# alibaba/animate-anything

Measured on AMD Instinct MI355X. Metric: UNet3D denoising steps/sec @16fx512x512 bs=1, higher is better.
Workload: dtype fp16; 1 GPU; animate_anything_512_v1.02 UNet3D (1413M params, seeded random init), 16 frames x 512x512, pipeline bs=1 per GPU (CFG batch 2, 17 frames inside), DPM-Solver++ step, hipGraph=on; clips_per_gpu=1, clips=1, parallelism=clip-sharded x1, collective=none

## Files before the change

animate_anything_amd/csrc/aa_api.hip:

```cpp
#include "aa_launch.h"

namespace aa { thread_local hipError_t g_lds_error = hipSuccess; }

static const char* aa_post_launch() {
    hipError_t e = hipGetLastError();
    if (e == hipSuccess && aa::g_lds_error != hipSuccess) { e = aa::g_lds_error; aa::g_lds_error = hipSuccess; }
    return e == hipSuccess ? nullptr : hipGetErrorString(e);
}
#define AA_POST_LAUNCH() aa_post_launch()

#include "aa_api_impl.h"
```

animate_anything_amd/csrc/aa_api_impl.h:

```cpp
#pragma once
#include <stdarg.h>
#include <stdio.h>
#include <stdlib.h>
#include "aa_mi355.h"
#include "kernels/conv_gemm.h"
#include "kernels/conv_gemm_dma.h"
#include "kernels/conv_slab.h"
#include "kernels/conv_gemm_x.h"
#include "kernels/norm.h"
#include "kernels/attention.h"
#include "kernels/seq_attention.h"
#include "kernels/ff_fused.h"
#include "kernels/linear_rows.h"
#include "kernels/linear_fp8.h"
#include "kernels/glue.h"

namespace aa {

static thread_local char g_err[512] = "";

static int fail(int code, const char* fmt, ...) {
    va_list ap;
    va_start(ap, fmt);
    vsnprintf(g_err, sizeof(g_err), fmt, ap);
    va_end(ap);
    return code;
}

static int finish(const char* what) {
    const char* e = AA_POST_LAUNCH();
    if (e) return fail(AA_E_HIP, "%s: %s", what, e);
    return AA_OK;
}

static bool aligned16(const void* p) { return (reinterpret_cast<uintptr_t>(p) & 15) == 0; }

struct CgCfg { int bm, bn, wm, wn, bk, stages, per_cu; float rate; int slab = 0; int x = 0; int sched = 0; };
constexpr int cg_dp(int dp3, int dp0, int dp1) { return (dp3 | dp0 << 4 | dp1 << 8) << 6; }
static const CgCfg kCgCfgs[] = {
    {128, 64, 2, 2, 64, 2, 3, 0.78f},
    {128, 128, 2, 2, 64, 2, 2, 0.90f},
    {192, 256, 3, 2, 64, 2, 1, 1.05f},
    {256, 256, 4, 2, 64, 2, 1, 1.10f},
    {256, 320, 4, 2, 64, 2, 1, 1.10f},
    {192, 320, 3, 2, 64, 2, 1, 1.05f},
    {256, 320, 4, 2, 32, 4, 1, 1.15f},
    {256, 256, 4, 2, 32, 4, 1, 1.15f},
    {128, 128, 2, 2, 32, 4, 2, 0.95f},
    {128, 64, 2, 2, 32, 4, 3, 0.80f},
    {192, 320, 3, 2, 32, 4, 1, 1.10f},
    {128, 320, 2, 2, 32, 2, 2, 1.10f},
    {128, 256, 2, 2, 32, 2, 2, 1.05f},
    {128, 256, 2, 2, 64, 2, 1, 1.00f},
    {256, 320, 4, 2, 64, 2, 1, 1.30f, 0, 0, 1},
    {256, 256, 4, 2, 64, 2, 1, 1.25f, 0, 0, 1},
    {128, 128, 2, 2, 32, 2, 3, 0.90f},
    {128, 64, 2, 2, 32, 2, 4, 0.78f},
    {64, 128, 2, 2, 32, 2, 4, 0.70f},
    {64, 64, 2, 2, 32, 2, 6, 0.60f},
    {64, 256, 2, 2, 32, 2, 3, 0.80f},
    {256, 320, 4, 2, 32, 4, 1, 1.20f, 0, 0, 1},
    {256, 256, 4, 2, 32, 4, 1, 1.20f, 0, 0, 1},
    {192, 256, 2, 4, 64, 2, 1, 1.05f},
    {192, 256, 2, 4, 64, 2, 1, 1.05f, 0, 0, 1},
    {128, 256, 2, 4, 32, 2, 2, 1.00f},
    {256, 320, 4, 2, 64, 2, 1, 1.30f, 0, 0, 2},
    {256, 256, 4, 2, 64, 2, 1, 1.25f, 0, 0, 2},
    {192, 256, 2, 4, 64, 2, 1, 1.05f, 0, 0, 2},
    {256, 320, 4, 2, 32, 4, 1, 1.20f, 0, 0, 2},
    {128, 320, 2, 2, 32, 2, 2, 1.10f, 0, 0, 2},
    {128, 128, 2, 2, 64, 2, 2, 0.90f, 0, 0, 2},
    {192, 320, 3, 2, 64, 2, 1, 1.05f, 0, 0, 2},
    {128, 256, 2, 2, 32, 2, 2, 1.05f, 0, 0, 2},
    {256, 320, 4, 2, 32, 3, 1, 1.00f, 1},
    {256, 256, 4, 2, 32, 3, 1, 1.00f, 1},
    {256, 256, 2, 2, 64, 2, 1, 1.45f, 0, 1, cg_dp(8, 8, 0)},
    {256, 320, 2, 2, 64, 2, 1, 1.45f, 0, 1, cg_dp(11, 7, 0)},
    {256, 256, 2, 2, 64, 2, 1, 1.40f, 0, 1, cg_dp(6, 5, 5)},
    {256, 320, 2, 2, 64, 2, 1, 1.40f, 0, 1, cg_dp(7, 6, 5)},
    {256, 256, 4, 2, 64, 2, 1, 1.35f, 0, 1, cg_dp(2, 2, 2)},
    {256, 256, 2, 2, 32, 4, 1, 1.50f, 0, 1, cg_dp(4, 0, 0)},
    {256, 320, 2, 2, 32, 4, 1, 1.50f, 0, 1, cg_dp(5, 0, 0)},
    {256, 256, 4, 2, 32, 4, 1, 1.45f, 0, 1, cg_dp(2, 0, 0)},
    {128, 256, 2, 2, 32, 3, 2, 1.20f, 0, 1, cg_dp(3, 0, 0)},
    {256, 128, 4, 1, 32, 3, 2, 1.20f, 0, 1, cg_dp(3, 0, 0)},
    {192, 256, 2, 2, 64, 2, 1, 1.30f, 0, 1, cg_dp(5, 5, 4)},
    {128, 128, 2, 2, 64, 2, 2, 1.00f, 0, 1, cg_dp(2, 2, 2)},
    {128, 128, 2, 2, 32, 4, 2, 1.00f, 0, 1, cg_dp(2, 0, 0)},
    {192, 320, 2, 2, 64, 2, 1, 1.35f, 0, 1, cg_dp(6, 5, 5)},
};
constexpr int kNumCgCfgs = sizeof(kCgCfgs) / sizeof(kCgCfgs[0]);

static thread_local int g_tile_override = -2;
static int cg_force_cfg() {
    if (g_tile_override == -2) { const char* e = getenv("AA_FORCE_CFG"); g_tile_override = e ? atoi(e) : -1; }
    return g_tile_override;
}

static bool cg_slab_ok(const AaConvGemm& d, const CgCfg& c) {
    const int hw = d.h_in * d.w_in;
    return d.kh == 3 && d.kw == 3 && d.stride == 1 && d.pad_h == 1 && d.pad_w == 1 && d.h_virt == d.h_in && d.w_virt == d.w_in &&
           d.h_out == d.h_in && d.w_out == d.w_in && d.k_order == 1 && d.c0 % 64 == 0 && d.c1 % 64 == 0 && !d.geglu && !d.bias_per_row &&
           c.bm % d.w_in == 0 && hw % c.bm == 0 && (c.bm / d.w_in + 2) * (d.w_in + 2) <= CS_SLAB_ROWS && !(d.debug & 8);
}

static thread_local unsigned g_x_disabled = 0;
static bool cg_x_ok(const AaConvGemm& d) {
    if (!(d.h_virt == d.h_in && d.w_virt == d.w_in)) return false;
    {
        const int taps = d.kh * d.kw;
        if (taps > 1 && d.k_order != 1) return false;
        if (taps > 31) return false;
        const int64_t px = (int64_t)d.n_img * d.h_in * d.w_in + (int64_t)d.pad_h * d.w_in + d.pad_w + (int64_t)d.kh * d.w_in + d.kw;
        if (px >= ((int64_t)1 << 24) || px * (d.c0 > d.c1 ? d.c0 : d.c1) * 2 >= ((int64_t)1 << 31)) return false;
    }
    if (d.rowvec) {
        const int64_t M = (int64_t)d.n_img * d.h_out * d.w_out;
        const int64_t ld = d.rowvec_ld ? d.rowvec_ld : d.n_out;
// ... 558 lines not shown
        AA_LAUNCH((groupnorm_coef_kernel<f16_t>), dim3(d->n_groups_img), dim3(GN_THREADS), lds, stream, *d, (const float*)ws, chunks, coef);
    } else {
        AA_LAUNCH((groupnorm_stats_kernel<bf16_t>), dim3(chunks, d->n_groups_img), dim3(GN_THREADS), (size_t)C * 8 * (1 + rpp), stream, *d, ws, chunks);
        AA_LAUNCH((groupnorm_coef_kernel<bf16_t>), dim3(d->n_groups_img), dim3(GN_THREADS), lds, stream, *d, (const float*)ws, chunks, coef);
    }
    return finish("groupnorm_coef");
}

int aa_layernorm(const void* x, const void* gamma, const void* beta, void* y, int64_t rows, int32_t channels,
                 float eps, int32_t dtype, void* stream) {
    using namespace aa;
    if (rows <= 0 || channels <= 0 || channels % 8 || channels > 2048) return fail(AA_E_SHAPE, "layernorm: rows=%lld channels=%d", (long long)rows, channels);
    if (!aligned16(x) || !aligned16(y) || !aligned16(gamma) || !aligned16(beta)) return fail(AA_E_ALIGN, "layernorm: operands must be 16-byte aligned");
    const int sj = channels <= 512 ? 1 : (channels <= 1024 ? 2 : 4);
    const int per_wg = 4 * (4 / sj);
    const dim3 grid((unsigned)((rows + per_wg - 1) / per_wg)), block(256);
    if (dtype != AA_F16 && dtype != AA_BF16) return fail(AA_E_DTYPE, "layernorm: unsupported dtype %d", dtype);
#define AA_LN(T, SJ) AA_LAUNCH((layernorm_kernel<T, SJ>), grid, block, 0, stream, (const T*)x, (const T*)gamma, (const T*)beta, (T*)y, rows, channels, eps)
    if (dtype == AA_F16) { if (sj == 1) AA_LN(f16_t, 1); else if (sj == 2) AA_LN(f16_t, 2); else AA_LN(f16_t, 4); }
    else                 { if (sj == 1) AA_LN(bf16_t, 1); else if (sj == 2) AA_LN(bf16_t, 2); else AA_LN(bf16_t, 4); }
#undef AA_LN
    return finish("layernorm");
}

int aa_ln_finalize(const float* stats, int32_t parts, float* coef, int64_t rows, int32_t channels, float eps, void* stream) {
    using namespace aa;
    if (!stats || !coef || parts <= 0 || rows <= 0 || channels <= 0) return fail(AA_E_SHAPE, "ln_finalize: rows=%lld parts=%d channels=%d", (long long)rows, parts, channels);
    if (!aligned16(coef)) return fail(AA_E_ALIGN, "ln_finalize: coef must be 16-byte aligned");
    const dim3 grid((unsigned)((rows + 255) / 256)), block(256);
    AA_LAUNCH(ln_finalize_kernel<0>, grid, block, 0, stream, stats, coef, rows, (int)parts, 1.0f / (float)channels, eps);
    return finish("ln_finalize");
}

int aa_attention(const AaAttention* d, void* stream) {
    using namespace aa;
    if (!d) return fail(AA_E_SHAPE, "attention: null descriptor");
    if (d->head_dim != 64 && d->head_dim != 8 && d->head_dim != 80) return fail(AA_E_SHAPE, "attention: head_dim must be 64, 8 or 80 (got %d)", d->head_dim);
    if (d->q_len <= 0 || d->kv_len <= 0 || d->heads <= 0 || d->n_outer <= 0 || d->n_inner <= 0) return fail(AA_E_SHAPE, "attention: bad lengths");
    const AaAttnOperand* ops[4] = {&d->q, &d->k, &d->v, &d->o};
    for (const AaAttnOperand* x : ops) {
        if (!aligned16(x->ptr) || x->ld % 8 || x->col0 % 8) return fail(AA_E_ALIGN, "attention: operand rows must be 16-byte aligned");
        if (x->outer_div <= 0) return fail(AA_E_SHAPE, "attention: outer_div must be >= 1");
        if (x->seq_mod < 0) return fail(AA_E_SHAPE, "attention: seq_mod must be >= 0");
    }
    if (d->q.seq_mod || d->o.seq_mod) return fail(AA_E_SHAPE, "attention: seq_mod addressing is for K / V only");
    if (d->causal && d->head_dim != 64) return fail(AA_E_SHAPE, "attention: causal masking is implemented for head_dim 64");
    if (d->head_dim == 64 && (attn_extent_bytes(d->k, d->n_outer, d->n_inner, d->kv_len) >= ((int64_t)1 << 31) ||
        attn_extent_bytes(d->v, d->n_outer, d->n_inner, d->kv_len) >= ((int64_t)1 << 31)))
        return fail(AA_E_SHAPE, "attention: K / V operand must stay below 2 GiB");
    if (d->dtype == AA_F16) return attention_t<f16_t>(*d, stream);
    if (d->dtype == AA_BF16) return attention_t<bf16_t>(*d, stream);
    return fail(AA_E_DTYPE, "attention: unsupported dtype %d", d->dtype);
}

int aa_seq_self_attention_ok(const AaSeqSelfAttn* d) {
    using namespace aa;
    if (!d) return 0;
    if (d->channels != 320 && d->channels != 512 && d->channels != 640) return 0;
    if (d->seq_len < 1 || d->seq_len > 32 || d->n_outer <= 0 || d->n_inner <= 0) return 0;
    if (d->ldx % 8 || d->ldo % 8 || d->ldx < d->channels || d->ldo < d->channels) return 0;
    if (d->x_bytes <= 0 || d->o_bytes <= 0 || d->x_bytes >= ((int64_t)1 << 31) || d->o_bytes >= ((int64_t)1 << 31)) return 0;
    if (d->dtype != AA_F16 && d->dtype != AA_BF16) return 0;
    return 1;
}

int aa_seq_self_attention(const AaSeqSelfAttn* d, void* stream) {
    using namespace aa;
    if (!d) return fail(AA_E_SHAPE, "seq_self_attention: null descriptor");
    if (!aa_seq_self_attention_ok(d))
        return fail(AA_E_SHAPE, "seq_self_attention: unsupported call (channels %d, seq_len %d, ldx %d, ldo %d, dtype %d)", d->channels, d->seq_len, d->ldx, d->ldo, d->dtype);
    if (!aligned16(d->x) || !aligned16(d->w) || !aligned16(d->o) || !aligned16(d->w_bias))
        return fail(AA_E_ALIGN, "seq_self_attention: operands must be 16-byte aligned");
    if (d->normalize && !(d->ln_eps > 0.0f)) return fail(AA_E_SHAPE, "seq_self_attention: normalize needs ln_eps > 0");
    if (d->pre_w) {
        if (!d->pre_out || !aligned16(d->pre_w) || !aligned16(d->pre_out) || !aligned16(d->pre_bias) || !aligned16(d->pre_residual))
            return fail(AA_E_ALIGN, "seq_self_attention: the projection in front needs pre_out and 16-byte aligned operands");
        const int64_t rows_ext = d->x_bytes / (2 * (int64_t)d->ldx);
        if (d->ld_pre % 8 || d->ld_pre < d->channels || rows_ext * d->ld_pre * 2 >= ((int64_t)1 << 31) ||
            (d->pre_residual && (d->ld_res % 8 || d->ld_res < d->channels || rows_ext * d->ld_res * 2 >= ((int64_t)1 << 31))))
            return fail(AA_E_SHAPE, "seq_self_attention: bad row pitch / extent of pre_out / pre_residual");
    } else if (d->pre_bias || d->pre_residual || d->pre_out) return fail(AA_E_SHAPE, "seq_self_attention: pre_bias / pre_residual / pre_out without pre_w");
    const int per = (32 * SA_NW) / d->seq_len;
    const int64_t n_seq = (int64_t)d->n_outer * d->n_inner;
    const dim3 grid((unsigned)((n_seq + per - 1) / per)), block(64 * SA_NW);
    const size_t lds = sa_lds_bytes(d->channels);
#define AA_SA(T, C_) AA_LAUNCH((seq_self_attention_kernel<T, C_>), grid, block, lds, stream, *d)
    if (d->dtype == AA_F16) {
        if (d->channels == 320) AA_SA(f16_t, 320); else if (d->channels == 512) AA_SA(f16_t, 512); else AA_SA(f16_t, 640);
    } else {
        if (d->channels == 320) AA_SA(bf16_t, 320); else if (d->channels == 512) AA_SA(bf16_t, 512); else AA_SA(bf16_t, 640);
    }
#undef AA_SA
    return finish("seq_self_attention");
}

int aa_ff_fused_ok(const AaFFFused* d) {
    if (!d || d->channels != 320 || d->rows <= 0) return 0;
    if (d->ldx % 8 || d->ldo % 8 || d->ld_outer % 8 || d->ldx < d->channels || d->ldo < d->channels || (d->outer && d->ld_outer < d->channels)) return 0;
    const int64_t lim = (int64_t)1 << 31;
    if (d->rows * d->ldx * 2 >= lim || d->rows * d->ldo * 2 >= lim || (d->outer && d->rows * d->ld_outer * 2 >= lim)) return 0;
    if (d->dtype != AA_F16 && d->dtype != AA_BF16) return 0;
    return 1;
}

int aa_ff_fused(const AaFFFused* d, void* stream) {
    using namespace aa;
    if (!d) return fail(AA_E_SHAPE, "ff_fused: null descriptor");
    if (!aa_ff_fused_ok(d)) return fail(AA_E_SHAPE, "ff_fused: unsupported call (channels %d, rows %lld, dtype %d)", d->channels, (long long)d->rows, d->dtype);
    if (!d->x || !d->out || !d->w) return fail(AA_E_SHAPE, "ff_fused: x, out, w are required");
    if (!aligned16(d->x) || !aligned16(d->outer) || !aligned16(d->out) || !aligned16(d->w)) return fail(AA_E_ALIGN, "ff_fused: operands must be 16-byte aligned");
    if (d->normalize && !(d->ln_eps > 0.0f)) return fail(AA_E_SHAPE, "ff_fused: normalize needs ln_eps > 0");
    const dim3 grid((unsigned)((d->rows + 32 * FF_NW - 1) / (32 * FF_NW))), block(64 * FF_NW);
    const int abl = d->flags >> 8;
#define AA_FF(ABL_) case ABL_: AA_LAUNCH((ff_fused_kernel<f16_t, 320, ABL_>), grid, block, ff_lds_bytes(), stream, *d); break
    if (abl && d->dtype == AA_F16) {
        switch (abl) { AA_FF(1); AA_FF(4); AA_FF(8); AA_FF(16); AA_FF(32); AA_FF(33); AA_FF(24); AA_FF(61); AA_FF(256); AA_FF(64); AA_FF(128); AA_FF(512);
                       default: return fail(AA_E_SHAPE, "ff_fused: no instantiation for ablation %d", abl); }
    } else if (d->dtype == AA_F16) AA_LAUNCH((ff_fused_kernel<f16_t, 320>), grid, block, ff_lds_bytes(), stream, *d);
    else                    AA_LAUNCH((ff_fused_kernel<bf16_t, 320>), grid, block, ff_lds_bytes(), stream, *d);
#undef AA_FF
    return finish("ff_fused");
}

int aa_linear_rows_ok(const AaLinearRows* d) {
    if (!d || d->channels != 320 || d->rows <= 0 || d->n_out <= 0 || d->n_out % 32) return 0;
    if (d->ldx % 8 || d->ldo % 8 || d->ld_res % 8 || d->ldx < d->channels || d->ldo < d->n_out || (d->residual && d->ld_res < d->n_out)) return 0;
    const int64_t lim = (int64_t)1 << 31;
    if (d->rows * d->ldx * 2 >= lim || d->rows * d->ldo * 2 >= lim || (d->residual && d->rows * d->ld_res * 2 >= lim)) return 0;
    if (d->dtype != AA_F16 && d->dtype != AA_BF16) return 0;
    if (d->row_affine && (d->rows_per_group <= 0 || d->rows_per_group % 32)) return 0;
    return 1;
}

int aa_linear_rows(const AaLinearRows* d, void* stream) {
    using namespace aa;
    if (!d) return fail(AA_E_SHAPE, "linear_rows: null descriptor");
    if (!aa_linear_rows_ok(d)) return fail(AA_E_SHAPE, "linear_rows: unsupported call (channels %d, n_out %d, rows %lld, dtype %d)", d->channels, d->n_out, (long long)d->rows, d->dtype);
    if (!d->x || !d->out || !d->w) return fail(AA_E_SHAPE, "linear_rows: x, out, w are required");
    if (!aligned16(d->x) || !aligned16(d->residual) || !aligned16(d->out) || !aligned16(d->w) || !aligned16(d->row_affine)) return fail(AA_E_ALIGN, "linear_rows: operands must be 16-byte aligned");
    if (d->normalize && !(d->ln_eps > 0.0f)) return fail(AA_E_SHAPE, "linear_rows: normalize needs ln_eps > 0");
    const int tiles = (int)((d->rows + 32 * LR_NW - 1) / (32 * LR_NW)), nq = d->n_out / 32;
    const int slots = ((d->flags & 1) ? 2 : 256) * 2;
    int n_full = (d->flags & 2) ? tiles : tiles / slots * slots, n_split = 1;
    if (tiles - n_full > 0)
        for (int s = 2; s <= nq && (tiles - n_full) * s <= slots; ++s)
            if (nq % s == 0) n_split = s;
    if (n_split == 1) n_full = tiles;
    const dim3 grid((unsigned)(n_full + (tiles - n_full) * n_split)), block(64 * LR_NW);
    if (d->dtype == AA_F16) AA_LAUNCH((linear_rows_kernel<f16_t, 320>), grid, block, lr_lds_bytes(), stream, *d, n_full, n_split);
    else                    AA_LAUNCH((linear_rows_kernel<bf16_t, 320>), grid, block, lr_lds_bytes(), stream, *d, n_full, n_split);
    return finish("linear_rows");
}

int aa_quant_rows_fp8(const AaQuantRowsFp8* d, void* stream) {
    using namespace aa;
    if (!d) return fail(AA_E_SHAPE, "quant_rows_fp8: null descriptor");
    if (d->rows <= 0 || d->channels <= 0 || d->channels % 16 || d->channels > 5120) return fail(AA_E_SHAPE, "quant_rows_fp8: rows=%lld channels=%d (a multiple of 16, at most 5120)", (long long)d->rows, d->channels);
    if (d->ldx % 8 || d->ldq % 16 || d->ldx < d->channels || d->ldq < d->channels) return fail(AA_E_SHAPE, "quant_rows_fp8: row pitches ldx=%d ldq=%d", d->ldx, d->ldq);
    if (!d->x || !d->q || !d->scale) return fail(AA_E_SHAPE, "quant_rows_fp8: x, q, scale are required");
    if (!aligned16(d->x) || !aligned16(d->q) || !aligned16(d->gamma) || !aligned16(d->beta)) return fail(AA_E_ALIGN, "quant_rows_fp8: operands must be 16-byte aligned");
    if (d->gamma && !(d->ln_eps > 0.0f)) return fail(AA_E_SHAPE, "quant_rows_fp8: LayerNorm needs ln_eps > 0");
    if (d->dtype != AA_F16 && d->dtype != AA_BF16) return fail(AA_E_DTYPE, "quant_rows_fp8: unsupported dtype %d", d->dtype);
    const dim3 grid((unsigned)((d->rows + 3) / 4)), block(256);
    const int pieces = (d->channels + 1023) / 1024;
#define AA_Q8(T, J) AA_LAUNCH((quant_rows_fp8_kernel<T, J>), grid, block, 0, stream, *d)
    if (d->dtype == AA_F16) { if (pieces <= 1) AA_Q8(f16_t, 1); else if (pieces == 2) AA_Q8(f16_t, 2); else if (pieces == 3) AA_Q8(f16_t, 3); else AA_Q8(f16_t, 5); }
    else                    { if (pieces <= 1) AA_Q8(bf16_t, 1); else if (pieces == 2) AA_Q8(bf16_t, 2); else if (pieces == 3) AA_Q8(bf16_t, 3); else AA_Q8(bf16_t, 5); }
#undef AA_Q8
    return finish("quant_rows_fp8");
}

int aa_linear_fp8(const AaLinearFp8* d, void* stream) {
    using namespace aa;
    if (!d) return fail(AA_E_SHAPE, "linear_fp8: null descriptor");
    if (d->rows <= 0 || d->n <= 0 || d->k <= 0 || d->k % 128 || d->n % 64) return fail(AA_E_SHAPE, "linear_fp8: rows=%lld n=%d k=%d (k a multiple of 128, n of 64)", (long long)d->rows, d->n, d->k);
    if (!d->a || !d->a_scale || !d->w || !d->w_scale || !d->out) return fail(AA_E_SHAPE, "linear_fp8: a, a_scale, w, w_scale, out are required");
    if (d->geglu && d->residual) return fail(AA_E_SHAPE, "linear_fp8: the geglu epilogue takes no residual");
    const int n_store = d->geglu ? d->n / 2 : d->n;
    if (d->ldo % 8 || d->ldo < n_store || (d->residual && (d->ld_res % 8 || d->ld_res < n_store))) return fail(AA_E_SHAPE, "linear_fp8: row pitches ldo=%d ld_res=%d", d->ldo, d->ld_res);
    const int64_t lim = (int64_t)1 << 31;
    if (d->rows * d->k >= lim || (int64_t)d->n * d->k >= lim || d->rows * d->ldo * 2 >= lim || (d->residual && d->rows * d->ld_res * 2 >= lim))
        return fail(AA_E_SHAPE, "linear_fp8: every operand must stay below 2 GiB");
    if (!aligned16(d->a) || !aligned16(d->w) || !aligned16(d->w_scale) || !aligned16(d->bias) || !aligned16(d->residual) || !aligned16(d->out))
        return fail(AA_E_ALIGN, "linear_fp8: operands must be 16-byte aligned");
    if (d->dtype != AA_F16 && d->dtype != AA_BF16) return fail(AA_E_DTYPE, "linear_fp8: unsupported dtype %d", d->dtype);
    const int tiles_m = (int)((d->rows + L8_BM - 1) / L8_BM), tiles_n = (d->n + L8_BN - 1) / L8_BN;
    const dim3 grid((unsigned)(tiles_m * tiles_n)), block(256);
    if (d->dtype == AA_F16) {
        if (d->geglu) AA_LAUNCH((linear_fp8_kernel<f16_t, true>), grid, block, L8_LDS_BYTES, stream, *d, tiles_m, tiles_n);
        else          AA_LAUNCH((linear_fp8_kernel<f16_t, false>), grid, block, L8_LDS_BYTES, stream, *d, tiles_m, tiles_n);
    } else {
        if (d->geglu) AA_LAUNCH((linear_fp8_kernel<bf16_t, true>), grid, block, L8_LDS_BYTES, stream, *d, tiles_m, tiles_n);
        else          AA_LAUNCH((linear_fp8_kernel<bf16_t, false>), grid, block, L8_LDS_BYTES, stream, *d, tiles_m, tiles_n);
    }
    return finish("linear_fp8");
}

int aa_softmax_rows(const float* x, void* y, int64_t rows, int32_t cols, int32_t x_ld, int32_t y_ld, int32_t dtype, void* stream) {
    using namespace aa;
    if (rows <= 0 || cols <= 0 || x_ld < cols || y_ld < cols) return fail(AA_E_SHAPE, "softmax_rows: bad shape");
    const dim3 grid((unsigned)rows), block(256);
    if (dtype == AA_F16) AA_LAUNCH((softmax_rows_kernel<f16_t>), grid, block, 64, stream, x, (f16_t*)y, cols, x_ld, y_ld);
    else if (dtype == AA_BF16) AA_LAUNCH((softmax_rows_kernel<bf16_t>), grid, block, 64, stream, x, (bf16_t*)y, cols, x_ld, y_ld);
    else return fail(AA_E_DTYPE, "softmax_rows: unsupported dtype %d", dtype);
    return finish("softmax_rows");
}

int aa_cfg_dpm_step(const AaDpmStep* d, void* stream) {
    using namespace aa;
    if (!d || d->n <= 0) return fail(AA_E_SHAPE, "cfg_dpm_step: bad size");
    int64_t blocks = (d->n + 255) / 256;
    if (blocks > 2048) blocks = 2048;
    const dim3 grid((unsigned)blocks), block(256);
    if (d->dtype == AA_F16) AA_LAUNCH((cfg_dpm_step_kernel<f16_t>), grid, block, 0, stream, *d);
    else if (d->dtype == AA_BF16) AA_LAUNCH((cfg_dpm_step_kernel<bf16_t>), grid, block, 0, stream, *d);
    else return fail(AA_E_DTYPE, "cfg_dpm_step: unsupported dtype %d", d->dtype);
    return finish("cfg_dpm_step");
}

int aa_timestep_embedding(const float* t, void* out, int32_t n, int32_t dim, int32_t dtype, void* stream) {
    using namespace aa;
    if (!t || !out || n <= 0 || dim <= 0 || dim % 2) return fail(AA_E_SHAPE, "timestep_embedding: n=%d dim=%d", n, dim);
    const dim3 grid((unsigned)((n * (dim / 2) + 255) / 256)), block(256);
    if (dtype == AA_F16) AA_LAUNCH((timestep_embed_kernel<f16_t>), grid, block, 0, stream, t, (f16_t*)out, n, dim);
    else if (dtype == AA_BF16) AA_LAUNCH((timestep_embed_kernel<bf16_t>), grid, block, 0, stream, t, (bf16_t*)out, n, dim);
    else return fail(AA_E_DTYPE, "timestep_embedding: unsupported dtype %d", dtype);
    return finish("timestep_embedding");
}

int aa_pack_latents(const AaPackLatents* d, void* stream) {
    using namespace aa;
// ... 86 lines not shown
```

animate_anything_amd/csrc/kernels/seq_attention.h:

```cpp
#pragma once
#include "dev.h"
#include "aa_mi355.h"

namespace aa {

constexpr int SA_NW = 4;
__host__ __device__ constexpr int sa_chunk_k(int channels) { return channels == 320 ? 32 : 64; }
__host__ __device__ constexpr int sa_stage_chunks(int channels) { return channels % 320 == 0 ? 5 : 4; }
__host__ __device__ constexpr int sa_per_cu(int channels) { return channels == 320 ? 2 : 1; }
__host__ __device__ constexpr int sa_lds_bytes(int channels) { return 2 * sa_stage_chunks(channels) * 128 * sa_chunk_k(channels) + SA_NW * 8192; }

__device__ __forceinline__ int64_t sa_seq_row(const AaSeqSelfAttn& p, int seq) {
    const int o = seq / p.n_inner, i = seq - o * p.n_inner;
    return (int64_t)o * p.outer_stride + (int64_t)i * p.inner_stride;
}

template <typename T, int C, int KC = sa_chunk_k(C), int SC = sa_stage_chunks(C), int PER_CU = sa_per_cu(C)>
__global__ void __launch_bounds__(64 * SA_NW, PER_CU) seq_self_attention_kernel(const AaSeqSelfAttn p) {
    constexpr int NW = SA_NW;
    constexpr int H = C / 64, NKS = C / 16, NKC = C / KC, SPP = NKC / SC;
    static_assert(C % 64 == 0 && NKC % SC == 0 && (KC == 64 || KC == 32), "channels");
    constexpr int CHUNK_BYTES = 128 * KC;
    constexpr int RB = 2 * KC;
    constexpr int SPR = KC / 8;
    constexpr int RPB = 256 / RB;
    constexpr int RPP = 1024 / RB;
    constexpr int PPC = 64 / RPP;
    constexpr int SPC = KC / 16;
    constexpr int STAGE_BYTES = SC * CHUNK_BYTES;
    constexpr int PIECES = SC * PPC, PPW = PIECES / NW;
    static_assert(PIECES % NW == 0, "DMA share");
    constexpr unsigned OOB = 0x80000000u;
    char* ring = dyn_smem();
    char* xch = ring + 2 * STAGE_BYTES;

    const int tid = threadIdx.x, lane = tid & 63;
    const int wave = wave_id();
    const int c = lane & 31, h = lane >> 5;
    const int L = p.seq_len;
    const int P = (32 * NW) / L;
    const int n_seq = p.n_outer * p.n_inner;
    const int s0 = blockIdx.x * P;
    const int rows_valid = min(P, n_seq - s0) * L;
    const bool wave_live = 32 * wave < rows_valid;

    const int r = 32 * wave + c;
    const bool row_ok = r < rows_valid;
    const int rs = r / L, rp = r - rs * L;
    const int64_t trow = row_ok ? sa_seq_row(p, s0 + rs) + (int64_t)rp * p.pos_stride : 0;
    const int key_lo = rs * L - 32 * (wave - 1) - 4 * h;
    const bool from_prev = rs * L < 32 * wave;
    const int key_lo_side = from_prev ? key_lo : key_lo - 64;

    const BufRsrc r_x = make_rsrc(p.x, (unsigned)p.x_bytes);
    const BufRsrc r_o = make_rsrc(p.o, (unsigned)p.o_bytes);
    const BufRsrc r_w = make_rsrc(p.w, (unsigned)((int64_t)H * 3 * 64 * C * 2));

    unsigned w_lane[PPW];
#pragma unroll
    for (int j = 0; j < PPW; ++j) {
        const int pi = wave + NW * j, kc = pi / PPC, rg = pi % PPC;
        const int row = RPP * rg + lane / SPR;
        const int slot = (lane % SPR) ^ ((row / RPB) & (SPR - 1));
        w_lane[j] = (unsigned)((row * C + kc * KC + slot * 8) * 2);
    }
    constexpr int NQH = H * 3 * SPP;
    const bool has_pre = p.pre_w != nullptr;
    const int NPRE = has_pre ? (C / 64) * SPP : 0;
    const int NQ = NPRE + NQH;
    const BufRsrc r_pw = make_rsrc(p.pre_w, has_pre ? (unsigned)((int64_t)C * C * 2) : 0u);
    auto issue = [&](int q, int buf) __attribute__((always_inline)) {
        const bool pre = q < NPRE;
        const int qq = pre ? q : q - NPRE;
        const int hp = qq / SPP, sub = qq - hp * SPP;
        const unsigned uni = (unsigned)((hp * 64 * C + sub * SC * KC) * 2);
#pragma unroll
        for (int j = 0; j < PPW; ++j) {
            const int pi = wave + NW * j;
            async_copy16_buf_s(pre ? r_pw : r_w, w_lane[j], uni, ring + buf * STAGE_BYTES + (pi / PPC) * CHUNK_BYTES + (pi % PPC) * 1024);
        }
    };
    const int dbg = p.flags;
    issue(0, 0);

    u32x4 xf[NKS];
    if (!wave_live) {
#pragma unroll
        for (int u = 0; u < 8; ++u) *reinterpret_cast<u32x4*>(xch + wave * 8192 + u * 1024 + lane * 16) = u32x4{0u, 0u, 0u, 0u};
    }

    unsigned wa[SPC];
#pragma unroll
    for (int v = 0; v < SPC; ++v) wa[v] = (unsigned)(c * RB + ((((v >> 1) * 4 + 2 * h + (v & 1)) ^ ((c / RPB) & (SPR - 1))) << 4));

    const float sl2e = p.scale * 1.4426950408889634f;
    f32x16 zero16;
#pragma unroll
    for (int e = 0; e < 16; ++e) zero16[e] = 0.0f;

    f32x16 acc[2];
    auto stage = [&](auto pass_, auto sub_, const char* st, const u32x4 (&xop)[NKS]) __attribute__((always_inline)) {
        constexpr int pass = decltype(pass_)::value, sub = decltype(sub_)::value;
        constexpr int NU = SPC * SC;
        u32x4 wf[3][2];
        const char* b4[SPC];
#pragma unroll
        for (int v = 0; v < SPC; ++v) b4[v] = st + wa[v];
        auto rd = [&](auto u_) __attribute__((always_inline)) {
            constexpr int u = decltype(u_)::value, kc = u / SPC, v = u % SPC, set = u % 3;
            lds_read16_async_off<kc * CHUNK_BYTES>(wf[set][0], b4[v]);
            lds_read16_async_off<kc * CHUNK_BYTES + 32 * RB>(wf[set][1], b4[v]);
        };
        rd(IntTag<0>());
        if constexpr (NU > 1) rd(IntTag<1>());
        static_for<NU>([&](auto u_) __attribute__((always_inline)) {
            constexpr int u = decltype(u_)::value, set = u % 3, ks = sub * SC * SPC + u;
            if constexpr (u + 2 < NU) { rd(IntTag<u + 2>()); lds_wait<4>(wf[set][0]); }
            else if constexpr (u + 1 < NU) lds_wait<2>(wf[set][0]);
            else lds_wait<0>(wf[set][0]);
            lds_pin(wf[set][1]);
#pragma unroll
            for (int j = 0; j < 2; ++j) {
                if constexpr (pass == 1) acc[j] = mfma_32x32x16(T(), xop[ks], wf[set][j], acc[j]);
                else                     acc[j] = mfma_32x32x16(T(), wf[set][j], xop[ks], acc[j]);
            }
        });
    };
    f32x16 pbias[2];
    auto fetch_bias = [&](auto pass_, const float* b) __attribute__((always_inline)) {
        constexpr int pass = decltype(pass_)::value;
        acc[0] = zero16; acc[1] = zero16;
        if (b == nullptr) { pbias[0] = zero16; pbias[1] = zero16; return; }
#pragma unroll
        for (int j = 0; j < 2; ++j) {
            if constexpr (pass == 1) {
                const float v = b[32 * j + c];
#pragma unroll
                for (int e = 0; e < 16; ++e) pbias[j][e] = v;
            } else {
#pragma unroll
                for (int g4 = 0; g4 < 4; ++g4) {
                    const f32x4 v = *reinterpret_cast<const f32x4*>(b + 32 * j + 8 * g4 + 4 * h);
#pragma unroll
                    for (int e = 0; e < 4; ++e) pbias[j][4 * g4 + e] = v[e];
                }
            }
        }
    };
    auto to_operands = [&](u32x4 (&op)[4]) __attribute__((always_inline)) {
#pragma unroll
        for (int j = 0; j < 2; ++j)
#pragma unroll
            for (int t = 0; t < 2; ++t) {
                Pack8<T> v;
#pragma unroll
                for (int e = 0; e < 8; ++e) v.e[e] = (T)(acc[j][8 * t + e] + pbias[j][8 * t + e]);
                op[2 * j + t] = v.raw;
            }
    };

    int q = 0;
    {
        const unsigned xb = (row_ok && !(dbg & 8)) ? (unsigned)(trow * p.ldx * 2) + (unsigned)(16 * h * 2) : OOB;
        if (has_pre) {
            u32x4 xin[NKS];
#pragma unroll
            for (int ks = 0; ks < NKS; ++ks) xin[ks] = buf_load16(r_x, xb + (unsigned)((32 * (ks >> 1) + 8 * (ks & 1)) * 2));
            const int64_t rows_ext = p.x_bytes / (2 * (int64_t)p.ldx);
            const BufRsrc r_res = make_rsrc(p.pre_residual, p.pre_residual ? (unsigned)(rows_ext * p.ld_res * 2) : 0u);
            const BufRsrc r_po = make_rsrc(p.pre_out, (unsigned)(rows_ext * p.ld_pre * 2));
            const unsigned rb = (row_ok && p.pre_residual) ? (unsigned)(trow * p.ld_res * 2) + (unsigned)(16 * h * 2) : OOB;
            const unsigned pb = (row_ok && !(dbg & 16)) ? (unsigned)(trow * p.ld_pre * 2) + (unsigned)(16 * h * 2) : OOB;
            static_for<C / 64>([&](auto pp_) __attribute__((always_inline)) {
                constexpr int pp = decltype(pp_)::value;
                u32x4 res[4];
                static_for<SPP>([&](auto sub_) __attribute__((always_inline)) {
                    if (sub_.value == 0 && pp > 0) lds_wait_all(); else mem_wait_all();
                    block_barrier();
                    if (q + 1 < NQ && !((dbg & 2) && q >= 1)) issue(q + 1, (q + 1) & 1);
                    if constexpr (sub_.value == 0) fetch_bias(IntTag<0>(), p.pre_bias ? p.pre_bias + pp * 64 : nullptr);
                    if constexpr (sub_.value == SPP - 1) {
#pragma unroll
                        for (int u = 0; u < 4; ++u) res[u] = buf_load16(r_res, rb + (unsigned)((64 * pp + 32 * (u >> 1) + 8 * (u & 1)) * 2));
                    }
                    if (wave_live && !(dbg & 4)) stage(IntTag<0>(), sub_, ring + (q & 1) * STAGE_BYTES, xin);
                    ++q;
                });
                dma_wait<0>();
#pragma unroll
                for (int j = 0; j < 2; ++j)
#pragma unroll
                    for (int t = 0; t < 2; ++t) {
                        Pack8<T> v; v.raw = res[2 * j + t];
#pragma unroll
                        for (int e = 0; e < 8; ++e) v.e[e] = (T)(acc[j][8 * t + e] + pbias[j][8 * t + e] + (float)v.e[e]);
                        buf_store16(r_po, pb + (unsigned)((64 * pp + 32 * j + 8 * t) * 2), v.raw);
                    }
            });
            dma_wait<0>();
            const unsigned pl = row_ok ? (unsigned)(trow * p.ld_pre * 2) + (unsigned)(16 * h * 2) : OOB;
#pragma unroll
            for (int ks = 0; ks < NKS; ++ks) xf[ks] = buf_load16(r_po, pl + (unsigned)((32 * (ks >> 1) + 8 * (ks & 1)) * 2));
        } else {
#pragma unroll
            for (int ks = 0; ks < NKS; ++ks) xf[ks] = buf_load16(r_x, xb + (unsigned)((32 * (ks >> 1) + 8 * (ks & 1)) * 2));
        }
    }
    if (p.normalize && !(dbg & (8 | 32))) {
        float sum = 0.0f;
#pragma unroll
        for (int ks = 0; ks < NKS; ++ks)
#pragma unroll
            for (int k = 0; k < 4; ++k) sum = dot2_f32(T(), xf[ks][k], ones_pair(T()), sum);
        const float mean = wave_sum_halves(sum) * (1.0f / (float)C);
        const f32x2 nmean2 = f32x2{-mean, -mean};
        f32x2 var2 = f32x2{0.0f, 0.0f};
#pragma unroll
        for (int ks = 0; ks < NKS; ++ks) {
            Pack8<T> v; v.raw = xf[ks];
#pragma unroll
            for (int e = 0; e < 8; e += 2) {
                const f32x2 d = f32x2{(float)v.e[e], (float)v.e[e + 1]} + nmean2;
                var2 = __builtin_elementwise_fma(d, d, var2);
            }
        }
        const float rstd = 1.0f / sqrtf(wave_sum_halves(var2[0] + var2[1]) * (1.0f / (float)C) + p.ln_eps);
        const f32x2 rstd2 = f32x2{rstd, rstd}, off2 = f32x2{-mean * rstd, -mean * rstd};
#pragma unroll
        for (int ks = 0; ks < NKS; ++ks) {
            Pack8<T> v; v.raw = xf[ks];
#pragma unroll
            for (int e = 0; e < 8; e += 2) {
                const f32x2 y = __builtin_elementwise_fma(f32x2{(float)v.e[e], (float)v.e[e + 1]}, rstd2, off2);
                v.e[e] = (T)y[0]; v.e[e + 1] = (T)y[1];
            }
            xf[ks] = v.raw;
        }
    }
    for (int head = 0; head < H; ++head) {
        u32x4 qop[4];
        static_for<3>([&](auto pass_) __attribute__((always_inline)) {
            constexpr int pass = decltype(pass_)::value;
            static_for<SPP>([&](auto sub_) __attribute__((always_inline)) {
                if (pass == 0 && sub_.value == 0 && (head > 0 || has_pre)) lds_wait_all(); else mem_wait_all();
                block_barrier();
                if (q + 1 < NQ && !((dbg & 2) && q >= 1)) issue(q + 1, (q + 1) & 1);
                if constexpr (sub_.value == 0) fetch_bias(pass_, p.w_bias ? p.w_bias + (head * 3 + pass) * 64 : nullptr);
                if (wave_live && !(dbg & 4)) stage(pass_, sub_, ring + (q & 1) * STAGE_BYTES, xf);
                ++q;
            });
            if (wave_live) {
                if constexpr (pass < 2) {
                    u32x4 op[4];
                    to_operands(op);
#pragma unroll
                    for (int u = 0; u < 4; ++u) *reinterpret_cast<u32x4*>(xch + wave * 8192 + (4 * pass + u) * 1024 + lane * 16) = op[u];
                } else to_operands(qop);
            }
        });
        if (!wave_live || (dbg & 1)) { dma_wait<0>(); continue; }
        f32x16 sacc[3];
        bool have[3];
        const char* xslot[3];
#pragma unroll
        for (int n = 0; n < 3; ++n) {
            const int kb = wave - 1 + n;
            have[n] = kb >= 0 && kb < NW && 32 * kb < rows_valid;
            xslot[n] = xch + (have[n] ? kb : wave) * 8192 + lane * 16;
            sacc[n] = zero16;
        }
        {
            u32x4 kf[3][4];
#pragma unroll
            for (int n = 0; n < 3; ++n) {
                lds_read16_async_off<0>(kf[n][0], xslot[n]);
                lds_read16_async_off<1024>(kf[n][1], xslot[n]);
                lds_read16_async_off<2048>(kf[n][2], xslot[n]);
                lds_read16_async_off<3072>(kf[n][3], xslot[n]);
            }
            static_for<3>([&](auto n_) __attribute__((always_inline)) {
                constexpr int n = decltype(n_)::value;
                lds_wait<4 * (2 - n)>(kf[n][0]);
                lds_pin(kf[n][1]); lds_pin(kf[n][2]); lds_pin(kf[n][3]);
                if (have[n]) {
#pragma unroll
                    for (int u = 0; u < 4; ++u) sacc[n] = mfma_32x32x16(T(), kf[n][u], qop[u], sacc[n]);
                }
            });
        }
        f32x16 side;
#pragma unroll
        for (int e = 0; e < 16; ++e) side[e] = from_prev ? sacc[0][e] : sacc[2][e];
        float mx = -1.0e30f;
#pragma unroll
        for (int e = 0; e < 16; ++e) {
            const int off = (e & 3) + 8 * (e >> 2);
            const bool ok_s = (unsigned)(off - key_lo_side) < (unsigned)L;
            const bool ok_o = (unsigned)(off + 32 - key_lo) < (unsigned)L;
            const float ts = ok_s ? side[e] * sl2e : -1.0e30f;
            const float to = ok_o ? sacc[1][e] * sl2e : -1.0e30f;
            side[e] = ts;
            sacc[1][e] = to;
            mx = fmaxf(mx, fmaxf(ts, to));
        }
        mx = wave_max_halves(mx);
        float ps = 0.0f;
        u32x4 pop[3][2];
#pragma unroll
        for (int t = 0; t < 2; ++t) {
            Pack8<T> pk_s, pk_o;
#pragma unroll
            for (int e = 0; e < 8; ++e) {
                const float p_s = fast_exp2(side[8 * t + e] - mx), p_o = fast_exp2(sacc[1][8 * t + e] - mx);
                ps += p_s + p_o;
                pk_s.e[e] = (T)p_s;
                pk_o.e[e] = (T)p_o;
            }
            pop[1][t] = pk_o.raw;
#pragma unroll
            for (int k = 0; k < 4; ++k) { pop[0][t][k] = from_prev ? pk_s.raw[k] : 0u; pop[2][t][k] = from_prev ? 0u : pk_s.raw[k]; }
        }
        const float inv = 1.0f / wave_sum_halves(ps);
        f32x16 oacc[2];
        oacc[0] = zero16; oacc[1] = zero16;
        {
            u32x4 vf[3][4];
#pragma unroll
            for (int n = 0; n < 3; ++n) {
                lds_read16_async_off<4096>(vf[n][0], xslot[n]);
// ... 32 lines not shown
```

animate_anything_amd/ops.py:

```python
from __future__ import annotations

import ctypes as C
import os
from dataclasses import dataclass
from typing import Optional

import torch

from . import _lib
from ._lib import (AA_ACT_GELU, AA_ACT_NONE, AA_ACT_QUICK_GELU, AA_ACT_SILU, AA_BF16, AA_F16, AA_F32, AaAttention, AaAttnOperand,
                   AaBlend, AaConvGemm, AaFFFused, AaLinearRows, AaLinearFp8, AaQuantRowsFp8, AaDpmStep, AaDpmStepTok, AaEulerStepTok, AaGroupNorm, AaPackFrames, AaPackLatents, AaSeqSelfAttn)

_DT = {torch.float16: AA_F16, torch.bfloat16: AA_BF16, torch.float32: AA_F32}

TRACE = None

AUTOTUNE = True
LAST_STAMPS = None
GN_PLANS = None
MAX_OPERAND_BYTES = 1 << 31
FORCE_TILE = -1
ATTN_FLAGS = int(os.environ.get("AA_ATTN_FLAGS", "0"))
if ATTN_FLAGS & ~13:
    raise RuntimeError(f"AA_ATTN_FLAGS={ATTN_FLAGS}: only bits 0 (value 1), 2 (value 4) and 3 (value 8) exist")
# ... 548 lines not shown
    d.c0, d.c1 = c0, c1
    d.n_groups_img, d.tokens_per_group, d.num_groups = n_groups_img, tokens_per_group, num_groups
    d.silu, d.dtype, d.eps = int(silu), _DT[x0.dtype], eps
    nbytes = lib.aa_groupnorm_workspace(C.byref(d))
    ws = torch.empty(max(nbytes // 4, 1), dtype=torch.float32, device=x0.device)
    two_pass = False
    if AUTOTUNE and x0.is_cuda:
        key = (-1, d.dtype, c0, c1, n_groups_img, tokens_per_group, num_groups, int(silu))
        _load_default_tile_cache()
        choice = _tile_cache.get(key)
        if choice is None and y.data_ptr() != x0.data_ptr() and not torch.cuda.is_current_stream_capturing():
            choice = _autotune_groupnorm(lib, d, ws, nbytes, _stream(x0), key)
        two_pass = bool(choice and choice[0])
    if two_pass:
        lib.aa_set_groupnorm_two_pass(1)
    try:
        if GN_PLANS is not None:
            info = (C.c_int32 * 4)()
            GN_PLANS.append(tuple(info) if lib.aa_groupnorm_plan(C.byref(d), info) else None)
        _run(lib.aa_groupnorm, C.byref(d), _ptr(ws), nbytes, _stream(x0))
    finally:
        if two_pass:
            lib.aa_set_groupnorm_two_pass(0)
    return y


def groupnorm_coef(x0: torch.Tensor, gamma: torch.Tensor, beta: torch.Tensor, n_groups_img: int, tokens_per_group: int, num_groups: int = 32,
                   eps: float = 1e-5) -> torch.Tensor:
    lib = _lib.get()
    _check(x0, gamma, beta)
    c0 = x0.shape[-1]
    d = AaGroupNorm()
    d.x0, d.x1, d.gamma, d.beta, d.y = _ptr(x0), None, _ptr(gamma), _ptr(beta), None
    d.c0, d.c1 = c0, 0
    d.n_groups_img, d.tokens_per_group, d.num_groups = n_groups_img, tokens_per_group, num_groups
    d.silu, d.dtype, d.eps = 0, _DT[x0.dtype], eps
    nbytes = lib.aa_groupnorm_workspace(C.byref(d))
    ws = torch.empty(max(nbytes // 4, 1), dtype=torch.float32, device=x0.device)
    coef = torch.empty(n_groups_img, 2, c0, dtype=torch.float32, device=x0.device)
    _run(lib.aa_groupnorm_coef, C.byref(d), _ptr(ws), nbytes, _ptr(coef), _stream(x0))
    return coef


def layernorm(x: torch.Tensor, gamma: torch.Tensor, beta: torch.Tensor, eps: float = 1e-5) -> torch.Tensor:
    lib = _lib.get()
    _check(x, gamma, beta)
    y = torch.empty_like(x)
    _run(lib.aa_layernorm, _ptr(x), _ptr(gamma), _ptr(beta), _ptr(y), x.shape[0], x.shape[1], eps,
         _DT[x.dtype], _stream(x))
    return y


def _operand(t: torch.Tensor, col0: int, outer_stride: int, inner_stride: int, pos_stride: int, outer_div: int = 1):
    o = AaAttnOperand()
    o.ptr, o.ld, o.col0 = _ptr(t), t.stride(0), col0
    o.outer_stride, o.inner_stride, o.pos_stride, o.outer_div = outer_stride, inner_stride, pos_stride, outer_div
    return o


def attention(q: torch.Tensor, q_col0: int, k: torch.Tensor, k_col0: int, v: torch.Tensor, v_col0: int,
              heads: int, n_outer: int, n_inner: int, q_len: int, kv_len: int,
              q_strides, kv_strides, kv_outer_div: int = 1, scale: Optional[float] = None, head_dim: int = 64,
              kv_seq_mod: int = 0, causal: bool = False) -> torch.Tensor:
    lib = _lib.get()
    for t in (q, k, v):
        if (not t.is_cuda and not _lib.host_pointers_ok()) or t.stride(-1) != 1:
            raise RuntimeError("attention: operands must be GPU tensors with contiguous rows")
    out = torch.empty(q.shape[0], heads * head_dim, dtype=q.dtype, device=q.device)
    d = AaAttention()
    d.q = _operand(q, q_col0, *q_strides)
    d.k = _operand(k, k_col0, *kv_strides, outer_div=kv_outer_div)
    d.v = _operand(v, v_col0, *kv_strides, outer_div=kv_outer_div)
    d.o = _operand(out, 0, *q_strides)
    d.k.seq_mod = d.v.seq_mod = kv_seq_mod
    d.causal = int(causal)
    d._pad = ATTN_FLAGS
    d.n_outer, d.n_inner, d.heads, d.head_dim = n_outer, n_inner, heads, head_dim
    d.q_len, d.kv_len, d.dtype = q_len, kv_len, _DT[q.dtype]
    d.scale = float(head_dim) ** -0.5 if scale is None else scale
    _run(lib.aa_attention, C.byref(d), _stream(q))
    return out


SEQ_ATTN_DEBUG = 0


@dataclass
class SeqQKV:
    w: torch.Tensor
    bias: Optional[torch.Tensor]
    ln_eps: float


def pack_seq_qkv(wq: torch.Tensor, wk: torch.Tensor, wv: torch.Tensor, ln=None) -> SeqQKV:
    n, c = wq.shape
    assert n % 64 == 0 and wk.shape == (n, c) and wv.shape == (n, c)
    i = torch.arange(32, device=wq.device)
    perm = 16 * ((i >> 2) & 1) + 4 * (i >> 3) + (i & 3)
    perm64 = torch.cat([perm, perm + 32])
    heads = n // 64

    def order(t):
        q, k, v = (t[j].reshape((heads, 64) + tuple(t.shape[2:])) for j in range(3))
        return torch.stack([k, v[:, perm64], q], dim=1).contiguous()

    w3 = torch.stack([wq.detach(), wk.detach(), wv.detach()])
    bias, eps = None, 0.0
    if ln is not None:
        gamma, beta, eps = ln
        wf = w3.float()
        bias = order(wf @ beta.detach().float())
        w3 = (wf * gamma.detach().float()[None, None, :]).to(wq.dtype)
    return SeqQKV(order(w3), bias, float(eps))


@dataclass
class SeqPre:
    w: torch.Tensor
    bias: Optional[torch.Tensor]


def pack_seq_pre(weight: torch.Tensor, bias: Optional[torch.Tensor] = None) -> SeqPre:
    n, c = weight.shape
    assert n == c and n % 64 == 0
    i = torch.arange(32, device=weight.device)
    perm = 16 * ((i >> 2) & 1) + 4 * (i >> 3) + (i & 3)
    rows = (torch.arange(0, n, 32, device=weight.device)[:, None] + perm[None, :]).reshape(-1)
    b = None if bias is None else bias.detach().float()[rows].contiguous()
    return SeqPre(weight.detach()[rows].reshape(n // 64, 64, c).contiguous(), b)


def _seq_self_attn_desc(x, pk, out, n_outer, n_inner, seq_len, strides, scale):
    d = AaSeqSelfAttn()
    d.x, d.w, d.w_bias, d.o = _ptr(x), _ptr(pk.w), _ptr(pk.bias), _ptr(out)
    d.outer_stride, d.inner_stride, d.pos_stride = strides
    last = (n_outer - 1) * strides[0] + (n_inner - 1) * strides[1] + (seq_len - 1) * strides[2]
    d.x_bytes, d.o_bytes = (last + 1) * x.stride(0) * 2, (last + 1) * out.stride(0) * 2
    d.n_outer, d.n_inner, d.seq_len, d.channels = n_outer, n_inner, seq_len, x.shape[1]
    d.ldx, d.ldo = x.stride(0), out.stride(0)
    d.normalize, d.ln_eps, d.scale, d.dtype = int(pk.ln_eps > 0.0), float(pk.ln_eps), float(scale), _DT[x.dtype]
    d.flags = SEQ_ATTN_DEBUG
    return d


def seq_self_attention_ok(channels: int, seq_len: int, rows: int, dtype) -> bool:
    d = AaSeqSelfAttn()
    d.channels, d.seq_len, d.n_outer, d.n_inner, d.ldx, d.ldo = channels, seq_len, 1, 1, channels, channels
    d.x_bytes = d.o_bytes = rows * channels * 2
    d.dtype = _DT.get(dtype, -1)
    return bool(_lib.get().aa_seq_self_attention_ok(C.byref(d)))


def seq_self_attention(x: torch.Tensor, pk: SeqQKV, n_outer: int, n_inner: int, seq_len: int, strides, scale: Optional[float] = None,
                       pre: Optional[SeqPre] = None, residual: Optional[torch.Tensor] = None):
    lib = _lib.get()
    _check(x, pk.w, pk.bias, residual)
    if pk.w.dtype != x.dtype or pk.w.shape[-1] != x.shape[1]:
        raise RuntimeError("seq_self_attention: weights were packed for another dtype / width")
    out = torch.empty(x.shape[0], x.shape[1], dtype=x.dtype, device=x.device)
    d = _seq_self_attn_desc(x, pk, out, n_outer, n_inner, seq_len, strides, 64.0 ** -0.5 if scale is None else scale)
    x_pre = None
    if pre is not None:
        _check(pre.w, pre.bias)
        if pre.w.dtype != x.dtype or pre.w.shape[-1] != x.shape[1]:
            raise RuntimeError("seq_self_attention: the projection in front was packed for another dtype / width")
        x_pre = torch.empty_like(out)
        d.pre_w, d.pre_bias, d.pre_residual, d.pre_out = _ptr(pre.w), _ptr(pre.bias), _ptr(residual), _ptr(x_pre)
# ... 383 lines not shown
```

Before: 16.57 steps/s.

## Split tail-wave tiles of seq self-attention across heads and query CU count

```diff
diff --git a/animate_anything_amd/csrc/aa_api.hip b/animate_anything_amd/csrc/aa_api.hip
--- a/animate_anything_amd/csrc/aa_api.hip
+++ b/animate_anything_amd/csrc/aa_api.hip
@@ -9,4 +9,16 @@
 }
 #define AA_POST_LAUNCH() aa_post_launch()
 
+static int aa_cu_count() {
+    static int cached[64] = {};
+    int dev = 0;
+    if (hipGetDevice(&dev) != hipSuccess || dev < 0 || dev >= 64) return 256;
+    if (cached[dev] == 0) {
+        int n = 0;
+        cached[dev] = (hipDeviceGetAttribute(&n, hipDeviceAttributeMultiprocessorCount, dev) == hipSuccess && n > 0) ? n : 256;
+    }
+    return cached[dev];
+}
+#define AA_CU_COUNT() aa_cu_count()
+
 #include "aa_api_impl.h"
diff --git a/animate_anything_amd/csrc/aa_api_impl.h b/animate_anything_amd/csrc/aa_api_impl.h
--- a/animate_anything_amd/csrc/aa_api_impl.h
+++ b/animate_anything_amd/csrc/aa_api_impl.h
@@ -3,6 +3,7 @@
 #include <stdio.h>
 #include <stdlib.h>
 #include "aa_mi355.h"
+#include "tail_plan.h"
 #include "kernels/conv_gemm.h"
 #include "kernels/conv_gemm_dma.h"
 #include "kernels/conv_slab.h"
@@ -34,6 +35,10 @@
 }
 
 static bool aligned16(const void* p) { return (reinterpret_cast<uintptr_t>(p) & 15) == 0; }
+
+#ifndef AA_CU_COUNT
+#define AA_CU_COUNT() 256
+#endif
 
 struct CgCfg { int bm, bn, wm, wn, bk, stages, per_cu; float rate; int slab = 0; int x = 0; int sched = 0; };
 constexpr int cg_dp(int dp3, int dp0, int dp1) { return (dp3 | dp0 << 4 | dp1 << 8) << 6; }
@@ -758,9 +763,12 @@
     } else if (d->pre_bias || d->pre_residual || d->pre_out) return fail(AA_E_SHAPE, "seq_self_attention: pre_bias / pre_residual / pre_out without pre_w");
     const int per = (32 * SA_NW) / d->seq_len;
     const int64_t n_seq = (int64_t)d->n_outer * d->n_inner;
-    const dim3 grid((unsigned)((n_seq + per - 1) / per)), block(64 * SA_NW);
+    const int tiles = (int)((n_seq + per - 1) / per);
+    const TailPlan pl = plan_seq_attention(tiles, d->channels / 64, (d->flags & 128) ? 2 : AA_CU_COUNT(), sa_per_cu(d->channels),
+                                           !(d->flags & 64) && !d->pre_w && d->channels != 640);
+    const dim3 grid((unsigned)pl.grid()), block(64 * SA_NW);
     const size_t lds = sa_lds_bytes(d->channels);
-#define AA_SA(T, C_) AA_LAUNCH((seq_self_attention_kernel<T, C_>), grid, block, lds, stream, *d)
+#define AA_SA(T, C_) AA_LAUNCH((seq_self_attention_kernel<T, C_>), grid, block, lds, stream, *d, pl.n_full, pl.n_split)
     if (d->dtype == AA_F16) {
         if (d->channels == 320) AA_SA(f16_t, 320); else if (d->channels == 512) AA_SA(f16_t, 512); else AA_SA(f16_t, 640);
     } else {
@@ -816,13 +824,9 @@
     if (!aligned16(d->x) || !aligned16(d->residual) || !aligned16(d->out) || !aligned16(d->w) || !aligned16(d->row_affine)) return fail(AA_E_ALIGN, "linear_rows: operands must be 16-byte aligned");
     if (d->normalize && !(d->ln_eps > 0.0f)) return fail(AA_E_SHAPE, "linear_rows: normalize needs ln_eps > 0");
     const int tiles = (int)((d->rows + 32 * LR_NW - 1) / (32 * LR_NW)), nq = d->n_out / 32;
-    const int slots = ((d->flags & 1) ? 2 : 256) * 2;
-    int n_full = (d->flags & 2) ? tiles : tiles / slots * slots, n_split = 1;
-    if (tiles - n_full > 0)
-        for (int s = 2; s <= nq && (tiles - n_full) * s <= slots; ++s)
-            if (nq % s == 0) n_split = s;
-    if (n_split == 1) n_full = tiles;
-    const dim3 grid((unsigned)(n_full + (tiles - n_full) * n_split)), block(64 * LR_NW);
+    const TailPlan pl = plan_linear_rows(tiles, nq, (d->flags & 1) ? 2 : AA_CU_COUNT(), !(d->flags & 2));
+    const int n_full = pl.n_full, n_split = pl.n_split;
+    const dim3 grid((unsigned)pl.grid()), block(64 * LR_NW);
     if (d->dtype == AA_F16) AA_LAUNCH((linear_rows_kernel<f16_t, 320>), grid, block, lr_lds_bytes(), stream, *d, n_full, n_split);
     else                    AA_LAUNCH((linear_rows_kernel<bf16_t, 320>), grid, block, lr_lds_bytes(), stream, *d, n_full, n_split);
     return finish("linear_rows");
diff --git a/animate_anything_amd/csrc/kernels/seq_attention.h b/animate_anything_amd/csrc/kernels/seq_attention.h
--- a/animate_anything_amd/csrc/kernels/seq_attention.h
+++ b/animate_anything_amd/csrc/kernels/seq_attention.h
@@ -1,6 +1,7 @@
 #pragma once
 #include "dev.h"
 #include "aa_mi355.h"
+#include "tail_plan.h"
 
 namespace aa {
 
@@ -16,7 +17,7 @@
 }
 
 template <typename T, int C, int KC = sa_chunk_k(C), int SC = sa_stage_chunks(C), int PER_CU = sa_per_cu(C)>
-__global__ void __launch_bounds__(64 * SA_NW, PER_CU) seq_self_attention_kernel(const AaSeqSelfAttn p) {
+__global__ void __launch_bounds__(64 * SA_NW, PER_CU) seq_self_attention_kernel(const AaSeqSelfAttn p, const int n_full, const int n_split) {
     constexpr int NW = SA_NW;
     constexpr int H = C / 64, NKS = C / 16, NKC = C / KC, SPP = NKC / SC;
     static_assert(C % 64 == 0 && NKC % SC == 0 && (KC == 64 || KC == 32), "channels");
@@ -40,7 +41,12 @@
     const int L = p.seq_len;
     const int P = (32 * NW) / L;
     const int n_seq = p.n_outer * p.n_inner;
-    const int s0 = blockIdx.x * P;
+    const int n_tail_wg = (int)gridDim.x - n_full;
+    const int over = (int)blockIdx.x < n_tail_wg ? (int)blockIdx.x : -1;
+    const int tile = over < 0 ? (int)blockIdx.x - n_tail_wg : n_full + over / n_split;
+    int h_lo = 0, h_hi = H;
+    if (over >= 0) seq_heads_of(H, over % n_split, n_split, h_lo, h_hi);
+    const int s0 = tile * P;
     const int rows_valid = min(P, n_seq - s0) * L;
     const bool wave_live = 32 * wave < rows_valid;
 
@@ -64,10 +70,10 @@
         const int slot = (lane % SPR) ^ ((row / RPB) & (SPR - 1));
         w_lane[j] = (unsigned)((row * C + kc * KC + slot * 8) * 2);
     }
-    constexpr int NQH = H * 3 * SPP;
     const bool has_pre = p.pre_w != nullptr;
     const int NPRE = has_pre ? (C / 64) * SPP : 0;
-    const int NQ = NPRE + NQH;
+    const int q_lo = h_lo * 3 * SPP;
+    const int NQ = NPRE + h_hi * 3 * SPP;
     const BufRsrc r_pw = make_rsrc(p.pre_w, has_pre ? (unsigned)((int64_t)C * C * 2) : 0u);
     auto issue = [&](int q, int buf) __attribute__((always_inline)) {
         const bool pre = q < NPRE;
@@ -81,7 +87,7 @@
         }
     };
     const int dbg = p.flags;
-    issue(0, 0);
+    issue(q_lo, q_lo & 1);
 
     u32x4 xf[NKS];
     if (!wave_live) {
@@ -159,7 +165,7 @@
             }
     };
 
-    int q = 0;
+    int q = q_lo;
     {
         const unsigned xb = (row_ok && !(dbg & 8)) ? (unsigned)(trow * p.ldx * 2) + (unsigned)(16 * h * 2) : OOB;
         if (has_pre) {
@@ -177,7 +183,7 @@
                 static_for<SPP>([&](auto sub_) __attribute__((always_inline)) {
                     if (sub_.value == 0 && pp > 0) lds_wait_all(); else mem_wait_all();
                     block_barrier();
-                    if (q + 1 < NQ && !((dbg & 2) && q >= 1)) issue(q + 1, (q + 1) & 1);
+                    if (q + 1 < NQ && !((dbg & 2) && q > q_lo)) issue(q + 1, (q + 1) & 1);
                     if constexpr (sub_.value == 0) fetch_bias(IntTag<0>(), p.pre_bias ? p.pre_bias + pp * 64 : nullptr);
                     if constexpr (sub_.value == SPP - 1) {
 #pragma unroll
@@ -237,14 +243,14 @@
             xf[ks] = v.raw;
         }
     }
-    for (int head = 0; head < H; ++head) {
+    for (int head = h_lo; head < h_hi; ++head) {
         u32x4 qop[4];
         static_for<3>([&](auto pass_) __attribute__((always_inline)) {
             constexpr int pass = decltype(pass_)::value;
             static_for<SPP>([&](auto sub_) __attribute__((always_inline)) {
-                if (pass == 0 && sub_.value == 0 && (head > 0 || has_pre)) lds_wait_all(); else mem_wait_all();
+                if (pass == 0 && sub_.value == 0 && (head > h_lo || has_pre)) lds_wait_all(); else mem_wait_all();
                 block_barrier();
-                if (q + 1 < NQ && !((dbg & 2) && q >= 1)) issue(q + 1, (q + 1) & 1);
+                if (q + 1 < NQ && !((dbg & 2) && q > q_lo)) issue(q + 1, (q + 1) & 1);
                 if constexpr (sub_.value == 0) fetch_bias(pass_, p.w_bias ? p.w_bias + (head * 3 + pass) * 64 : nullptr);
                 if (wave_live && !(dbg & 4)) stage(pass_, sub_, ring + (q & 1) * STAGE_BYTES, xf);
                 ++q;
diff --git a/animate_anything_amd/csrc/tail_plan.h b/animate_anything_amd/csrc/tail_plan.h
--- /dev/null
+++ b/animate_anything_amd/csrc/tail_plan.h
@@ -0,0 +1,38 @@
+#pragma once
+
+#if defined(__HIPCC__)
+#define AA_PLAN_HD __host__ __device__
+#else
+#define AA_PLAN_HD
+#endif
+
+namespace aa {
+
+struct TailPlan {
+    int n_full;
+    int n_tail;
+    int n_split;
+    int grid() const { return n_full + n_tail * n_split; }
+};
+
+inline TailPlan plan_tail_split(int tiles, int slots, int max_split, bool divisors, bool enabled) {
+    TailPlan pl{tiles, 0, 1};
+    if (!enabled || slots <= 0) return pl;
+    const int n_full = tiles / slots * slots, n_tail = tiles - n_full;
+    if (n_tail <= 0) return pl;
+    int s_best = 1;
+    for (int s = 2; s <= max_split && n_tail * s <= slots; ++s)
+        if (!divisors || max_split % s == 0) s_best = s;
+    if (s_best == 1) return pl;
+    return TailPlan{n_full, n_tail, s_best};
+}
+
+inline TailPlan plan_linear_rows(int tiles, int nq, int cus, bool enabled) { return plan_tail_split(tiles, 2 * cus, nq, true, enabled); }
+
+inline TailPlan plan_seq_attention(int tiles, int heads, int cus, int per_cu, bool enabled) { return plan_tail_split(tiles, per_cu * cus, heads, false, enabled); }
+AA_PLAN_HD inline void seq_heads_of(int heads, int part, int n_split, int& lo, int& hi) {
+    lo = part * heads / n_split;
+    hi = (part + 1) * heads / n_split;
+}
+
+}
diff --git a/animate_anything_amd/ops.py b/animate_anything_amd/ops.py
--- a/animate_anything_amd/ops.py
+++ b/animate_anything_amd/ops.py
@@ -654,7 +654,7 @@
     return out
 
 
-SEQ_ATTN_DEBUG = 0
+SEQ_ATTN_DEBUG = int(os.environ.get("AA_SEQ_ATTN_FLAGS", "0"))
 
 
 @dataclass
```

Measured after the change: 16.60 steps/s, median of 6. No clear change (+0.2%).
